# sandialabs/PyNucleus

Measured on AMD Instinct MI355X. Metric: element-pairs/sec assembled (2D P1 fractional s=0.5, dense) + % fp64 roofline, higher is better.
Workload: dtype f64; 1 GPU; 2D unit disc (uniform_disc refined 7x, 98304 cells), P1, 48769 DoFs, fractional s=0.5, horizon=inf, dense getDense incl. zeroExterior; 4831887360 element pairs/step; noRef=7, num_dofs=48769, num_cells=98304, parallelism=block rows of the upper triangle dealt over 1 GPU(s), row-owned one-sided slabs

## Files before the change

include/pnl_hip.h:

```cpp
#ifndef PNL_HIP_H
#define PNL_HIP_H
#include <stdint.h>

#ifdef __cplusplus
extern "C" {
#endif

typedef struct pnl_context pnl_context;

enum pnl_status {
    PNL_OK = 0,
    PNL_ERR_INVALID = -1,
    PNL_ERR_UNSUPPORTED = -2,
    PNL_ERR_HIP = -3,
    PNL_ERR_STATE = -4,
    PNL_ERR_ORDER = -5
};

enum pnl_kernel_type { PNL_FRACTIONAL = 0, PNL_INDICATOR = 1, PNL_PERIDYNAMIC = 2, PNL_GAUSSIAN = 3, PNL_EXPONENTIAL = 4,
                       PNL_GAUSSIAN_BOUNDARY = 5, PNL_EXPONENTIAL_BOUNDARY = 6 };

typedef struct {
    int32_t ktype;
    int32_t interaction;
// ... 48 lines not shown
int pnl_set_classes(pnl_context *ctx, int nclasses, int num_labels, const int32_t *cell_labels_host,
                    const int32_t *facet_labels_host, const int32_t *cls_of_host);
int pnl_set_nonsymmetric(pnl_context *ctx, int on);
int pnl_select_class(pnl_context *ctx, int k);
int pnl_set_kernel(pnl_context *ctx, int which, const pnl_kernel *kernel);
int pnl_set_order_formula(pnl_context *ctx, int which, const pnl_order_formula *formula);
int pnl_upload_distant_rules(pnl_context *ctx, int qmax, const int32_t *off_host, const double *bary_host,
                             const double *w_host, const double *phi_host, const int32_t *foff_host,
                             const double *fbary_host, const double *fw_host);
int pnl_upload_singular_rule(pnl_context *ctx, int which, int panel, int M, int rows, const double *nodes_host,
                             const double *w_host, const double *psi_host, double fac);
int pnl_upload_boundary(pnl_context *ctx, int nb, const int32_t *bcells_host);

int pnl_assemble_pairs_in_horizon(pnl_context *ctx, double *data, double *diag);
int pnl_assemble_pairs_in_horizon_range(pnl_context *ctx, double *data_dev, double *diag_dev, int cell_begin, int cell_end);

#define PNL_FLAG_NO_MIRROR 1
#define PNL_FLAG_SYMMETRIC_FLUSH 2
int pnl_assemble_dense(pnl_context *ctx, double *A_dev, int64_t ldA, int zero_exterior, int cell_begin, int cell_end,
                       int flags);
int pnl_block_row_costs(pnl_context *ctx, double *cost_out, int n);
int pnl_dense_overwrites(pnl_context *ctx, int cell_begin, int cell_end, int flags);
int pnl_tile_cells(pnl_context *ctx);
int pnl_assemble_dense_tiles(pnl_context *ctx, double *A_dev, int64_t ldA, int zero_exterior, int ntiles,
                             const int32_t *tiles_host, int cell_begin, int cell_end, int flags);
int pnl_upload_sparsity(pnl_context *ctx, int nnz, const int32_t *indptr_host, const int32_t *indices_host);
int pnl_upload_sparsity_device(pnl_context *ctx, int nnz, const int32_t *indptr_dev, const int32_t *indices_dev);
int pnl_assemble_pairs_masked(pnl_context *ctx, int np, const int32_t *pairs_host, const uint64_t *masks_host,
                              double *data_dev, double *diag_dev);
int pnl_assemble_boundary_masked(pnl_context *ctx, int ni, const int32_t *cells_host, const int32_t *facets_host,
                                 const uint32_t *masks_host, double fac, double *data_dev, double *diag_dev);
typedef struct {
    int32_t npairs, nnodes, nchunks, chunk_stride, ntiles, num_dslots, nfacets, tile;
    const int32_t *pair_nodes, *node_off, *node_dofs;
    const int32_t *chunk_cells, *chunk_ndof, *chunk_dofs;
    const int16_t *chunk_slot;
    const int32_t *tile_chunkA, *tile_chunkB, *tile_pair, *tile_flags, *tile_dslotA, *tile_dslotB;
    const int32_t *d_cell, *d_pair;
    int32_t n_sing[3];
    int32_t n_btouch;
    const int32_t *sing_items[3];
    const int32_t *pair_foff, *fvid;
    const int32_t *bt_slot, *bt_cell, *bt_facet;
} pnl_cluster_plan;
int pnl_assemble_clusters_tiled(pnl_context *ctx, const pnl_cluster_plan *plan, int cluster_boundary, double *data_dev,
                                double *diag_dev);
// ... 174 lines not shown
```

pynucleus_amd/_lib.py:

```python
import ctypes as C
import os
import numpy as np

_HERE = os.path.dirname(os.path.abspath(__file__))
LIB_PATH = os.environ.get('PNL_LIB', os.path.join(_HERE, 'libpnl_hip.so'))

PNL_OK = 0
PNL_ERR_INVALID = -1
PNL_ERR_UNSUPPORTED = -2
PNL_ERR_HIP = -3
PNL_ERR_STATE = -4
PNL_ERR_ORDER = -5
PNL_INTERIOR = 0
PNL_BOUNDARY = 1
PNL_FLAG_NO_MIRROR = 1
PNL_FLAG_SYMMETRIC_FLUSH = 2
PNL_NUM_COUNTERS = 134

EXPORTS = ['pnl_create', 'pnl_destroy', 'pnl_error_string', 'pnl_version', 'pnl_set_stream', 'pnl_synchronize',
           'pnl_upload_mesh', 'pnl_upload_dofmap', 'pnl_set_kernel', 'pnl_set_order_formula', 'pnl_upload_distant_rules',
           'pnl_upload_singular_rule', 'pnl_upload_boundary', 'pnl_assemble_dense', 'pnl_dense_overwrites', 'pnl_block_row_costs', 'pnl_tile_cells',
           'pnl_assemble_dense_tiles', 'pnl_get_counters', 'pnl_get_phase_ms', 'pnl_get_kernel_ms', 'pnl_tree_build', 'pnl_tree_build_blocks', 'pnl_tree_build_refined', 'pnl_tree_build_horizon', 'pnl_tree_build_device', 'pnl_tree_destroy', 'pnl_tree_sizes', 'pnl_tree_get', 'pnl_tree_node_cells', 'pnl_h2_transfer_matrices', 'pnl_nfplan_build', 'pnl_nfplan_destroy', 'pnl_nfplan_sizes', 'pnl_nfplan_get', 'pnl_horizon_pattern', 'pnl_near_pattern', 'pnl_pattern_set_max_nnz', 'pnl_set_option', 'pnl_set_cell_order', 'pnl_set_interaction_transform', 'pnl_set_order_vertex_values', 'pnl_h2_get', 'pnl_h2_set', 'pnl_pattern_nnz', 'pnl_pattern_get', 'pnl_pattern_destroy', 'pnl_set_row_slab', 'pnl_diag_blocks_size', 'pnl_get_diag_blocks', 'pnl_slab_matvec', 'pnl_slab_diagonal', 'pnl_gemv', 'pnl_cg_jacobi',
           'pnl_inv_diagonal', 'pnl_set_classes', 'pnl_select_class', 'pnl_upload_sparsity', 'pnl_upload_sparsity_device', 'pnl_assemble_pairs_masked', 'pnl_assemble_boundary_masked', 'pnl_assemble_clusters_tiled', 'pnl_h2_setup', 'pnl_h2_matvec', 'pnl_h2_upward', 'pnl_h2_interact', 'pnl_h2_downward', 'pnl_h2_sizes', 'pnl_spmv',
           'pnl_assemble_pairs_in_horizon', 'pnl_assemble_pairs_in_horizon_range', 'pnl_set_nonsymmetric', 'pnl_set_order_function', 'pnl_upload_pointwise_rules', 'pnl_assemble_dense_pointwise',
           'pnl_assemble_pairs_masked_pointwise', 'pnl_assemble_boundary_masked_pointwise',
           'pnl_gemv_axpby', 'pnl_csr_matvec', 'pnl_mg_create', 'pnl_mg_destroy', 'pnl_mg_cycle', 'pnl_mg_solve', 'pnl_mg_cg', 'pnl_theta_step', 'pnl_selftest',
           'pnl_potrf', 'pnl_potrs', 'pnl_getrf', 'pnl_getrs',
           'pnl_csr_cg_jacobi', 'pnl_fe_space_create', 'pnl_fe_space_destroy', 'pnl_assemble_nonlinearity', 'pnl_imex_create',
           'pnl_imex_destroy', 'pnl_imex_sweep']

PNL_FUN_BRUSSELATOR, PNL_FUN_CUBIC = 0, 1
PNL_IMEX_CG_MG, PNL_IMEX_CHOL = 0, 1
PNL_IMEX_MAX_STAGES, PNL_IMEX_MAX_COMP = 4, 2


def source_sha16():
    import glob
    import hashlib
    root = os.path.dirname(_HERE)
    files = sorted(glob.glob(os.path.join(_HERE, 'csrc', '*.h'))+glob.glob(os.path.join(_HERE, 'csrc', '*.hip'))
                   +[os.path.join(root, 'include', 'pnl_hip.h'), os.path.join(_HERE, 'csrc', 'Makefile')])
    h = hashlib.sha256()
    for fn in files:
        with open(fn, 'rb') as f:
# ... 68 lines not shown
    import torch
    L = C.CDLL(LIB_PATH)
    vp, i32, i64, dbl = C.c_void_p, C.c_int, C.c_int64, C.c_double
    L.pnl_create.argtypes = [i32, C.POINTER(vp)]
    L.pnl_destroy.argtypes = [vp]
    L.pnl_destroy.restype = None
    L.pnl_error_string.argtypes = [vp]
    L.pnl_error_string.restype = C.c_char_p
    L.pnl_version.restype = C.c_char_p
    L.pnl_set_stream.argtypes = [vp, vp]
    L.pnl_synchronize.argtypes = [vp]
    L.pnl_upload_mesh.argtypes = [vp, i32, i32, vp, i32, vp, vp, vp, dbl]
    L.pnl_upload_dofmap.argtypes = [vp, i32, i32, i32, i32, vp, vp]
    L.pnl_set_kernel.argtypes = [vp, i32, C.POINTER(pnl_kernel)]
    L.pnl_selftest.argtypes = [i32, i32, i32, i32, vp, i32, vp, vp]
    L.pnl_set_order_formula.argtypes = [vp, i32, C.POINTER(pnl_order_formula)]
    L.pnl_upload_distant_rules.argtypes = [vp, i32, vp, vp, vp, vp, vp, vp, vp]
    L.pnl_upload_singular_rule.argtypes = [vp, i32, i32, i32, i32, vp, vp, vp, dbl]
    L.pnl_upload_boundary.argtypes = [vp, i32, vp]
    L.pnl_assemble_dense.argtypes = [vp, vp, i64, i32, i32, i32, i32]
    L.pnl_dense_overwrites.argtypes = [vp, i32, i32, i32]
    L.pnl_block_row_costs.argtypes = [vp, vp, i32]
    L.pnl_tile_cells.argtypes = [vp]
    L.pnl_assemble_dense_tiles.argtypes = [vp, vp, i64, i32, i32, vp, i32, i32, i32]
    L.pnl_get_counters.argtypes = [vp, vp, i32]
    L.pnl_get_phase_ms.argtypes = [vp, vp, i32]
    L.pnl_get_kernel_ms.argtypes = [vp, vp, i32]
    L.pnl_set_row_slab.argtypes = [vp, i32, vp, i32, vp]
    L.pnl_tree_build.argtypes = [i32, i32, vp, vp, vp, i32, dbl, i32, i32, i32, C.POINTER(vp)]
    L.pnl_tree_build_blocks.argtypes = [i32, i32, vp, vp, vp, i32, dbl, i32, i32, i32, vp, i32, C.POINTER(vp)]
    L.pnl_tree_build_refined.argtypes = [i32, i32, vp, vp, vp, i32, dbl, i32, i32, i32, vp, i32, i32, C.POINTER(vp)]
    L.pnl_tree_build_horizon.argtypes = [i32, i32, vp, vp, vp, i32, dbl, i32, i32, i32, vp, i32, i32, dbl, C.POINTER(vp)]
    L.pnl_tree_build_device.argtypes = [i32, i32, vp, vp, vp, i32, dbl, i32, i32, i32, i32, C.POINTER(vp)]
    L.pnl_tree_destroy.argtypes = [vp]
    L.pnl_tree_destroy.restype = None
    L.pnl_tree_sizes.argtypes = [vp, vp]
    L.pnl_tree_get.argtypes = [vp, vp, vp, vp, vp, vp, vp, vp, vp]
    L.pnl_tree_node_cells.argtypes = [vp, i32, vp, vp, vp]
    L.pnl_h2_transfer_matrices.argtypes = [i32, i32, i32, vp, vp, vp]
    L.pnl_nfplan_build.argtypes = [i32, i32, vp, i32, vp, i32, i32, vp, i32, vp, vp, vp, vp, i32, vp, i32, i32, C.POINTER(vp)]
    L.pnl_nfplan_destroy.argtypes = [vp]
    L.pnl_nfplan_destroy.restype = None
    L.pnl_nfplan_sizes.argtypes = [vp, vp]
    L.pnl_nfplan_get.argtypes = [vp, i32, vp]
    L.pnl_horizon_pattern.argtypes = [i32, i32, vp, i32, vp, i32, i32, vp, dbl, i32, C.POINTER(vp)]
    L.pnl_near_pattern.argtypes = [vp, i32, vp, i32, C.POINTER(vp)]
# ... 242 lines not shown

    def set_stream(self, stream_ptr):
        self.check(self.L.pnl_set_stream(self.h, C.c_void_p(stream_ptr)))

    def synchronize(self):
        self.check(self.L.pnl_synchronize(self.h))

    def assemble_dense(self, A_ptr, ldA, zero_exterior, cell_begin, cell_end, flags=0):
        self.assembly_epoch = getattr(self, 'assembly_epoch', 0)+1
        self.check(self.L.pnl_assemble_dense(self.h, C.c_void_p(A_ptr), int(ldA), int(bool(zero_exterior)), int(cell_begin),
                                             int(cell_end), int(flags)))

    def block_row_costs(self, num_blocks):
        out = np.zeros(int(num_blocks))
        self.check(self.L.pnl_block_row_costs(self.h, out.ctypes.data, int(num_blocks)))
        return out

    def dense_overwrites(self, cell_begin, cell_end, flags=0):
        rc = self.L.pnl_dense_overwrites(self.h, int(cell_begin), int(cell_end), int(flags))
        if rc < 0:
            self.check(rc)
        return rc == 1

    def tile_cells(self):
        rc = self.L.pnl_tile_cells(self.h)
        if rc <= 0:
            self.check(rc)
        return rc

    def assemble_dense_tiles(self, A_ptr, ldA, zero_exterior, tiles, cell_begin, cell_end, flags=0):
        self.assembly_epoch = getattr(self, 'assembly_epoch', 0)+1
        t, pt = _hp(tiles, np.int32)
        self.check(self.L.pnl_assemble_dense_tiles(self.h, C.c_void_p(A_ptr), int(ldA), int(bool(zero_exterior)), t.shape[0], pt,
                                                   int(cell_begin), int(cell_end), int(flags)))

    def upload_sparsity(self, indptr, indices):
        ip, pip = _hp(indptr, np.int32)
        ix, pix = _hp(indices, np.int32)
        self.check(self.L.pnl_upload_sparsity(self.h, ix.shape[0], pip, pix))

    def upload_sparsity_device(self, indptr_t, indices_t):
        self.check(self.L.pnl_upload_sparsity_device(self.h, int(indices_t.numel()), C.c_void_p(indptr_t.data_ptr()),
                                                     C.c_void_p(indices_t.data_ptr()) if indices_t.numel() else None))

    def assemble_pairs_masked(self, pairs, masks, data_ptr, diag_ptr=None):
        p, pp = _hp(pairs, np.int32)
# ... 228 lines not shown
```

pynucleus_amd/csrc/pnl_context.h:

```cpp
#pragma once
#include <hip/hip_runtime.h>
#include <algorithm>
#include <cmath>
#include <cstdarg>
#include <cstdio>
#include <cstring>
#include <string>
#include <vector>
#include "pnl_hip.h"
#include "pnl_device.h"


constexpr int TILE_P1 = 64;
constexpr int TILE_P2 = 32;

struct DevBuf {
    void *p = nullptr;
    size_t bytes = 0;
    ~DevBuf() { release(); }
    void release() { if (p) { (void)hipFree(p); p = nullptr; bytes = 0; } }
};


struct pnl_context {
// ... 24 lines not shown
        int n_spairs[3] = {0, 0, 0}, n_bpairs[2] = {0, 0};
        int n_spairs1[3] = {0, 0, 0};
        ClassData() { std::memset(kern, 0, sizeof(kern)); std::memset(form, 0, sizeof(form)); }
    };
    std::vector<ClassData*> cls;
    int cur = 0;
    ClassData &C() { return *cls[cur]; }
    int nlab = 0;
    bool nonsym = false;
    int orient = 0;
    std::vector<int32_t> cell_labels, facet_labels, cls_of;
    bool have_mesh = false, have_dofs = false, have_rules = false, have_boundary = false;
    bool dirty = true;
    DevProblem P;
    DevBuf b_cellv, b_ccen, b_cvol, b_ch, b_clog, b_cvid, b_cdof, b_cslot, b_blk_ndof, b_blk_dofs, b_perm, b_off, b_bary, b_w, b_phi,
        b_foff, b_fbary, b_fw, b_bvid, b_bv, b_bgeo, b_counters, b_D, b_tiles,
        b_vec[6], b_clabel, b_blabel, b_clsof, b_scal, b_wl, b_wlcount, b_tilectr, b_ttn, b_ttoff, b_tttab, b_ttwphi, b_wlsorted, b_wlaux,
        b_vertices, b_sp_indptr, b_sp_indices, b_mp_pairs, b_mp_masks, b_mp_wl, b_mp_sorted, b_mp_aux, b_bi_cells, b_bi_facets,
        b_bi_masks, b_cp[28], b_cpD, b_wlds, b_wlpair, b_h2[20];
    DevBuf b_kcls, b_fcls, b_uni, b_tilecls, b_ttwphif;
    DevBuf b_scolbase, b_srowoff, b_cpoff, b_cpslot, b_cprow, b_foldtab, b_bkcls, b_bfcls, b_bdefer, b_multitiles, b_slotA, b_candtiles, b_candq;
    int slot_S = 0, n_multitiles = 0;
    long long slot_total = 0;
    DevBuf b_rowmap, b_rowdof, b_colmap, b_coldof;
    DevBuf b_cholinfo;
    DevBuf b_luwork, b_lutmp;
    std::vector<int32_t> slab_rowdofs, slab_coldofs;
    int slab_rows = 0, slab_cols = 0;
    bool slot_full_list = false;
    bool slot_used = false;
    std::vector<DevKernel> kcls_host;
    std::vector<DevKernel> bkcls_host;
    std::vector<DevFormula> bfcls_host;
    std::vector<DevFormula> fcls_host;
    int uni_off[5] = {-1, -1, -1, -1, -1}, uni_np[5] = {0, 0, 0, 0, 0};
    bool uni_struct[5] = {false, false, false, false, false};
    H2Dev h2;
    bool have_h2 = false;
    bool have_tile_order = false;
    struct TileOrderJob *tile_job = nullptr;
    DevBuf b_cellv_t, b_cdof_t, b_cslot_t, b_Dt;
    PwDev pw;
    bool have_pw = false, have_pw_rules[2][3] = {{false, false, false}, {false, false, false}};
    int pw_nkeys[2] = {0, 0};
    std::vector<double> pw_cell_smax, pw_facet_smax;
    std::vector<double> pw_vertex_s;
// ... 205 lines not shown
```

pynucleus_amd/csrc/pnl_device.h:

```cpp
#pragma once
#include <hip/hip_runtime.h>
#include <stdint.h>

#define PNL_NTHREADS 256
#define PNL_MAXQ 120
#define PNL_NCOUNTERS 134
#define PNL_WL_SLOTS 256

struct DevKernel {
    int ktype;
    int fast;
    double exponent, scale, horizon2;
    int interaction, qm;
    double pb[6];
    const double *ptab;
};

struct DevFormula {
    double c0, a, b, e, den0;
    int clip;
    int pad;
};

struct DevProblem {
// ... 30 lines not shown
    const double *sNodes[3], *sW[3], *sPsi[3];
    double sFac;
    int bM[2];
    const double *bNodes[2], *bW[2], *bPhi[2];
    double bFac;
    const int *bvid;
    const double *bv;
    const double *bgeo;
    const int *clabel, *blabel, *cls_of;
    int nlab, cur_class;
    int orient, pad2;
    double idfac;
    unsigned long long *counters;
    const int *rowmap, *colmap;
    int onesided, pad3;
    const double *uni = nullptr;
    int uni_off[5] = {0, 0, 0, 0, 0};
    int mix_struct = 0;
};

__device__ __forceinline__ long long pnl_row(const DevProblem &P, int I) { return P.rowmap ? (long long)P.rowmap[I] : (long long)I; }
__device__ __forceinline__ int pnl_col(const DevProblem &P, int J) { return P.colmap ? P.colmap[J] : J; }

#define PNL_FOLD_TAB 63
struct FoldEntry { long long off; int ar, cy; };

struct H2Dev {
    int dim, m, M, nnodes, nleaves, nfar;
    const double *box;
    const int *parent;
    const int *leaf_node;
    const int *leaf_dof_off, *leaf_dofs;
    const int *leaf_cell_off, *leaf_cells;
    const long long *leaf_val_off;
    const int *far;
    double *V, *K;
    const double *T;
    double *cup, *cdown;
};

__device__ __forceinline__ double cheb_node(double a, double b, int m, int j) {
    return (b-a)*0.5*(cos((2.0*(m-j)-1.0)/(2.0*m)*3.14159265358979323846)+1.0)+a;
}

__device__ __forceinline__ double lagrange1d(double a, double b, int m, int l, double x) {
    const double xl = cheb_node(a, b, m, l);
    double v = 1.;
    for (int k = 0; k < m; k++)
// ... 37 lines not shown
```

pynucleus_amd/csrc/pnl_hip.hip:

```cpp
#include <hip/hip_runtime.h>
#include <algorithm>
#include <cmath>
#include <cstdarg>
#include <cstdio>
#include <cstring>
#include <string>
#include <vector>
#include "pnl_hip.h"
#include "pnl_kernels.h"
#include "pnl_bndtile.h"

#include <thread>
#include "pnl_context.h"
#include "pnl_launch.h"

struct TileOrderJob {
    std::vector<int> cells, lperm;
    int nc = 0, T = 0, nblocks = 0, ncp = 0, dim = 0, dpe = 0;
    std::vector<double> cellv;
    std::vector<int32_t> cdof;
    std::vector<int16_t> cslot;
    std::thread worker;
};

namespace {


// ... 334 lines not shown
        for (int b = 0; b < nblocks; b++) colbase[b+1] = colbase[b]+((blk_ndof[b]+7) & ~7);
        const int S = colbase[nblocks];
        std::vector<long long> rowoff(nblocks, 0);
        long long run = 0;
        for (int a = 0; a < nblocks; a++) { rowoff[a] = run; run += (long long)blk_ndof[a]*(S-colbase[a]); }
        ctx->slot_S = S; ctx->slot_total = run;
        std::vector<int32_t> cpoff(ctx->N+1, 0);
        for (int b = 0; b < nblocks; b++) for (int g : lists[b]) cpoff[g+1]++;
        for (int g = 0; g < ctx->N; g++) cpoff[g+1] += cpoff[g];
        std::vector<int2> cp(cpoff[ctx->N]);
        std::vector<int32_t> fillp(cpoff.begin(), cpoff.end()-1);
        std::vector<long long> cprow(cp.size());
        for (int b = 0; b < nblocks; b++)
            for (size_t r = 0; r < lists[b].size(); r++) {
                const int k = fillp[lists[b][r]]++;
                cp[k] = make_int2(b, colbase[b]+(int)r);
                cprow[k] = rowoff[b]+(long long)r*(S-colbase[b])-colbase[b];
            }
        if ((rc = upload(ctx, ctx->b_cprow, cprow.data(), cprow.size()))) return rc;
        if ((rc = upload(ctx, ctx->b_scolbase, colbase.data(), colbase.size()))) return rc;
        if ((rc = upload(ctx, ctx->b_srowoff, rowoff.data(), rowoff.size()))) return rc;
        if ((rc = upload(ctx, ctx->b_cpoff, cpoff.data(), cpoff.size()))) return rc;
        if ((rc = upload(ctx, ctx->b_cpslot, cp.data(), cp.size()))) return rc;
        const int nranges = (ctx->N+31)/32;
        std::vector<FoldEntry> tab((size_t)nranges*(PNL_FOLD_TAB+1));
        for (int q = 0; q < nranges; q++) {
            FoldEntry *e = &tab[(size_t)q*(PNL_FOLD_TAB+1)];
            const int g0 = cpoff[q*32], g1 = cpoff[std::min(ctx->N, q*32+32)];
            e[0].off = g1-g0; e[0].ar = 0; e[0].cy = 0;
            if (g1-g0 > PNL_FOLD_TAB) continue;
            for (int I = q*32; I < std::min(ctx->N, q*32+32); I++)
                for (int g = cpoff[I]; g < cpoff[I+1]; g++) {
                    FoldEntry &x = e[1+g-g0];
                    x.off = cprow[g]; x.ar = (cp[g].x << 5) | (I-q*32); x.cy = cp[g].y;
                }
        }
        if ((rc = upload(ctx, ctx->b_foldtab, tab.data(), tab.size()))) return rc;
    }
    if ((rc = upload(ctx, ctx->b_perm, ctx->perm_table.data(), ctx->perm_table.size()))) return rc;
    const bool fresh_counters = !ctx->b_counters.p;
    if ((rc = ensure(ctx, ctx->b_counters, sizeof(unsigned long long)*PNL_NCOUNTERS))) return rc;
    if (fresh_counters) HIPCHK(ctx, hipMemset(ctx->b_counters.p, 0, sizeof(unsigned long long)*PNL_NCOUNTERS));
    if ((rc = ensure(ctx, ctx->b_D, sizeof(double)*(size_t)ncp*(dpe*(dpe+1)/2)))) return rc;

    DevProblem &P = ctx->P;
    P.dim = dim; P.dpe = dpe; P.nc = nc; P.ncp = ncp; P.N = ctx->N; P.dpv = ctx->dpv; P.dped = ctx->dped; P.nb = ctx->nb;
    P.H0 = ctx->H0;
    P.cellv = (const double*)ctx->b_cellv.p; P.ccen = (const double*)ctx->b_ccen.p;
    P.cvol = (const double*)ctx->b_cvol.p; P.ch = (const double*)ctx->b_ch.p; P.clog = (const double*)ctx->b_clog.p;
    P.cvid = (const int*)ctx->b_cvid.p; P.cdof = (const int*)ctx->b_cdof.p; P.cslot = (const short*)ctx->b_cslot.p;
    P.blk_ndof = (const int*)ctx->b_blk_ndof.p; P.blk_dofs = (const int*)ctx->b_blk_dofs.p;
    P.blk_stride = nU; P.nblocks = nblocks;
    P.perm_table = (const int*)ctx->b_perm.p;
    P.bvid = (const int*)ctx->b_bvid.p; P.bv = (const double*)ctx->b_bv.p; P.bgeo = (const double*)ctx->b_bgeo.p;
    P.counters = (unsigned long long*)ctx->b_counters.p;
    P.nlab = nlab; P.cur_class = -1; P.orient = 0; P.pad2 = 0; P.idfac = 1.;
    P.clabel = (const int*)ctx->b_clabel.p; P.blabel = (const int*)ctx->b_blabel.p; P.cls_of = (const int*)ctx->b_clsof.p;
    ctx->dirty = false;
    return PNL_OK;
// ... 889 lines not shown
        const double l_self = std::log(dmax/S.hmin), n_other = std::log(dmax/O.hmin);
        const double aL = std::min(F.a*O.Lmin, F.a*O.Lmax);
        const double bL = std::min(F.b*std::max(S.Lmin, O.Lmin), F.b*std::max(S.Lmax, O.Lmax));
        const double num = F.c0+aL+bL-F.e*n_other, den = l_self+F.den0;
        return den > 0. && num >= q*den*(1.+1e-9)+1e-9;
    };
    for (int q = 2; q <= qlimit; q++)
        if (upper(A, B, q) && upper(B, A, q)) {
            if (q == 2) return 2;
            return (lower(A, B, q-1) || lower(B, A, q-1)) ? q : 0;
        }
    return 0;
}

#include <deque>
#include <map>
#include <mutex>
namespace {
std::mutex g_opt_mutex;
std::map<std::string, const std::string*> g_options;
std::deque<std::string> g_option_values;
const char *const k_product_options[] = {"PNL_WL_FRAC", "PNL_FH_NOTILES", "PNL_NO_POWTAB", "PNL_VERBOSE", "PNL_PLAN_TIMING", "PNL_PLAN_THREADS", "PNL_BND_OLD",
                                         "PNL_NO_OVERLAP", "PNL_NO_FORK",
                                         "PNL_TILE_WGS", "PNL_UNI_GENERIC", "PNL_MIXED_GENERIC"};
}

const char *pnl_tune(const char *name) {
    {
        std::lock_guard<std::mutex> lk(g_opt_mutex);
        auto it = g_options.find(name);
        if (it != g_options.end()) return it->second->c_str();
    }
#ifdef PNL_TUNING
    return getenv(name);
#else
    return nullptr;
#endif
}

extern "C" {

const char *pnl_version(void) {
#ifdef PNL_TUNING
    return "pnl_hip 0.1 (gfx950, tuning build)";
#else
    return "pnl_hip 0.1 (gfx950)";
#endif
// ... 364 lines not shown
        if ((rc = upload(ctx, ctx->C().b_sn[slot], nodes, (size_t)2*nV*M))) return rc;
        if ((rc = upload(ctx, ctx->C().b_sw[slot], w, (size_t)M))) return rc;
        if ((rc = upload(ctx, ctx->C().b_sp[slot], psi, (size_t)rows*M))) return rc;
        ctx->C().sM[slot] = M; ctx->C().sRows[slot] = rows; ctx->C().sFac = facv;
    } else {
        if (rows != dpe) return fail(ctx, PNL_ERR_INVALID, "boundary singular rule has %d rows, expected %d", rows, dpe);
        if ((rc = upload(ctx, ctx->C().b_bn[slot], nodes, (size_t)(nV+dim)*M))) return rc;
        if ((rc = upload(ctx, ctx->C().b_bw[slot], w, (size_t)M))) return rc;
        if ((rc = upload(ctx, ctx->C().b_bp[slot], psi, (size_t)rows*M))) return rc;
        ctx->C().bM[slot] = M; ctx->C().bFac = facv;
    }
    ctx->C().have_sing[which][slot] = true;
    return PNL_OK;
}

int pnl_upload_boundary(pnl_context *ctx, int nb, const int32_t *bcells) {
    if (!ctx) return PNL_ERR_INVALID;
    if (!ctx->have_mesh) return fail(ctx, PNL_ERR_STATE, "upload the mesh first");
    if (nb < 0 || (nb > 0 && !bcells)) return fail(ctx, PNL_ERR_INVALID, "bad boundary arguments");
    ctx->nb = nb;
    ctx->bcells.assign(bcells, bcells+(size_t)nb*ctx->dim);
    ctx->have_boundary = true;
    ctx->dirty = true;
    return PNL_OK;
}

int pnl_tile_cells(pnl_context *ctx) {
    if (!ctx) return PNL_ERR_INVALID;
    int rc = finalize(ctx);
    return rc ? rc : ctx->tile;
}

static int upload_tiles(pnl_context *ctx, std::vector<int2> &tiles, int cell_begin, int cell_end) {
    const int ncls = (int)ctx->cls.size();
    std::vector<pnl_order_formula> forms(ncls);
    for (int k = 0; k < ncls; k++) forms[k] = ctx->cls[k]->form[0];
    if (tiles.size() == ctx->tiles_cached.size() && ctx->b_tiles.p && ctx->tiles_cb == cell_begin && ctx->tiles_ce == cell_end &&
        forms.size() == ctx->tiles_forms.size() && std::memcmp(forms.data(), ctx->tiles_forms.data(), sizeof(pnl_order_formula)*ncls) == 0 &&
        ctx->tiles_filter == ctx->tile_cell_filter &&
        (tiles.empty() || std::memcmp(tiles.data(), ctx->tiles_cached.data(), tiles.size()*sizeof(int2)) == 0))
        return PNL_OK;
    const int T = ctx->tile;
    const bool filter = ctx->tile_cell_filter;
    const bool p1 = T == 64 && (ctx->dpe == 3 || ctx->dpe == 2), p2 = ctx->dim == 2 && ctx->dpe == 6;
    const bool allow = ctx->use_pure && (p1 || p2) && ctx->qmax >= 2 && !ctx->nonsym;
    int qlimit = 2;
// ... 554 lines not shown
```

pynucleus_amd/csrc/pnl_tile2.h:

```cpp
#pragma once
#include "pnl_common.h"

__host__ __device__ constexpr int uni_rule_size(int dpe, int np) { return 3*np+np+np*dpe+(dpe*(dpe+1)/2)*np; }


#ifndef PNL_FOLD_FLAT
#define PNL_FOLD_FLAT 1
#endif
template <bool NT>
__global__ void __launch_bounds__(256)
k_fold_mirror(const double *__restrict__ A2, const FoldEntry *__restrict__ tab, const int *__restrict__ cpoff, const int2 *__restrict__ cp,
              const long long *__restrict__ cprow, double *__restrict__ A, long long ldA, int N) {
    __shared__ double t1[32][33], t2[32][33];
    __shared__ FoldEntry s_tab[2][PNL_FOLD_TAB+1];
    const unsigned nb = (unsigned)(N+31)/32;
    const unsigned nbs = (nb+7)/8;
    const unsigned sbid = blockIdx.x >> 6, inner = blockIdx.x & 63;
    unsigned I;
    {
        const float t = 2.f*(float)nbs+1.f;
        const float fb = (t-sqrtf(fmaxf(t*t-8.f*(float)sbid, 0.f)))*0.5f;
        I = (unsigned)fmaxf(fb, 0.f);
        if (I >= nbs) I = nbs-1;
        while (I > 0 && I*nbs-I*(I-1)/2 > sbid) I--;
        while (I+1 < nbs && (I+1)*nbs-(I+1)*I/2 <= sbid) I++;
    }
    const unsigned J = I+(sbid-(I*nbs-I*(I-1)/2));
    const unsigned bi = 8*I+(inner >> 3), bj = 8*J+(inner & 7);
    if (bi > bj || bj >= nb) return;
    const int tid = threadIdx.x, tx = tid & 31, ty = tid >> 5;
    if (tid < 2*(PNL_FOLD_TAB+1)) {
        const int side = tid >= PNL_FOLD_TAB+1, k = tid-side*(PNL_FOLD_TAB+1);
        s_tab[side][k] = tab[(size_t)(side ? bj : bi)*(PNL_FOLD_TAB+1)+k];
    }
    for (int k = tid; k < 32*33; k += 256) { (&t1[0][0])[k] = 0.; (&t2[0][0])[k] = 0.; }
    __syncthreads();
    const int n0 = (int)s_tab[0][0].off, n1 = (int)s_tab[1][0].off;
    if (n0 <= PNL_FOLD_TAB && n1 <= PNL_FOLD_TAB) {
#if PNL_FOLD_FLAT
#pragma unroll
        for (int g = 0; g < 2; g++) {
            if (g && bi == bj) break;
            const int nr = g ? n1 : n0, nc = g ? n0 : n1;
            double *__restrict__ tf = g ? &t2[0][0] : &t1[0][0];
            const unsigned total = (unsigned)(nr*nc), inv = ((1u << 20)+(unsigned)nc-1u)/(unsigned)nc;
            for (unsigned base = 0; base < total; base += 8*256) {
                double v[8];
                int dst[8];
#pragma unroll
                for (int u = 0; u < 8; u++) {
                    const unsigned idx = base+256u*u+(unsigned)tid;
                    dst[u] = -1;
                    v[u] = 0.;
                    if (idx < total) {
                        const unsigned ci = (idx*inv) >> 20, cj = idx-ci*(unsigned)nc;
                        const FoldEntry rw = s_tab[g][1+ci], col = s_tab[1-g][1+cj];
                        if ((col.ar >> 5) >= (rw.ar >> 5)) { v[u] = A2[rw.off+col.cy]; dst[u] = (rw.ar & 31)*33+(col.ar & 31); }
                    }
                }
#pragma unroll
                for (int u = 0; u < 8; u++) if (dst[u] >= 0) lds_add_f64(tf+dst[u], v[u]);
            }
        }
#else
#pragma unroll
        for (int g = 0; g < 2; g++) {
            if (g && bi == bj) break;
            const int nr = g ? n1 : n0, nc = g ? n0 : n1;
            double *__restrict__ tf = g ? &t2[0][0] : &t1[0][0];
            for (int cj = tx; cj < nc; cj += 32) {
                const FoldEntry col = s_tab[1-g][1+cj];
                const int cb = col.ar >> 5, c = col.ar & 31;
                for (int ci0 = ty; ci0 < nr; ci0 += 48) {
                    double v[6];
                    int dst[6];
#pragma unroll
                    for (int u = 0; u < 6; u++) {
                        const int ci = ci0+8*u;
                        dst[u] = -1;
                        v[u] = 0.;
                        if (ci < nr) {
                            const FoldEntry rw = s_tab[g][1+ci];
                            if (cb >= (rw.ar >> 5)) { v[u] = A2[rw.off+col.cy]; dst[u] = (rw.ar & 31)*33+c; }
                        }
                    }
#pragma unroll
                    for (int u = 0; u < 6; u++) if (dst[u] >= 0) lds_add_f64(tf+dst[u], v[u]);
                }
            }
        }
#endif
    } else {
        auto gather = [&](int br, int bc, double (*t)[33]) {
            const int J = min(bc*32+tx, N), j0 = cpoff[J], j1 = cpoff[min(J+1, N)];
#pragma unroll 1
            for (int rr = 0; rr < 4; rr++) {
                const int r = ty+8*rr, I = min(br*32+r, N);
                double s = 0.;
                for (int ci = cpoff[I]; ci < cpoff[min(I+1, N)]; ci++) {
                    const int a = cp[ci].x;
                    const double *__restrict__ rowp = A2+cprow[ci];
                    for (int cj = j0; cj < j1; cj++) {
                        const int2 c2 = cp[cj];
                        if (c2.x >= a) s += rowp[c2.y];
                    }
                }
                t[r][tx] = s;
            }
        };
        gather((int)bi, (int)bj, t1);
        if (bi != bj) gather((int)bj, (int)bi, t2);
    }
    __syncthreads();
    for (int r = ty; r < 32; r += 8) {
        const int I = bi*32+r, J = bj*32+tx;
        if (I < N && J < N) {
            const double v = (bi != bj) ? t1[r][tx]+t2[tx][r] : ((r != tx) ? t1[r][tx]+t1[tx][r] : t1[r][tx]);
            if (NT) __builtin_nontemporal_store(v, A+(long long)I*ldA+J); else A[(long long)I*ldA+J] = v;
        }
        const int I2 = bj*32+r, J2 = bi*32+tx;
        if (bi != bj && I2 < N && J2 < N) {
            const double v = t2[r][tx]+t1[tx][r];
            if (NT) __builtin_nontemporal_store(v, A+(long long)I2*ldA+J2); else A[(long long)I2*ldA+J2] = v;
        }
    }
}

__global__ void __launch_bounds__(256)
k_zero_slot_tiles(const SlotOut SO, const int2 *__restrict__ tiles, const int *__restrict__ blk_ndof) {
    const int a = tiles[blockIdx.x].x, b = tiles[blockIdx.x].y;
    const int nA = blk_ndof[a], nBp = SO.colbase[b+1]-SO.colbase[b], W = SO.S-SO.colbase[a];
    double *__restrict__ base = SO.A2+SO.rowoff[a]+(SO.colbase[b]-SO.colbase[a]);
    for (int t = threadIdx.x; t < nA*nBp; t += 256) {
        const int r = t/nBp, c = t-r*nBp;
        base[(long long)r*W+c] = 0.;
    }
}

__host__ __device__ constexpr size_t uniform_fixed_lds(int dpe, int np, int tile, int nUe, bool dof_lists = true) {
    return dpe == 3 ? sizeof(double)*(size_t)(2*tile*(np*2+1)+2*tile+2*tile*(np|1)+(dpe*(dpe+1)/2)*np)
                      +sizeof(int)*(size_t)(2*tile*(dpe|1)+2*tile+(dof_lists ? 4*nUe : 0))
                    : sizeof(double)*(size_t)(tile*np*2+tile*6+2*tile+2*tile*np+(dpe*(dpe+1)/2)*np)
                      +sizeof(int)*(size_t)(2*tile*dpe+2*tile+(dof_lists ? 4*nUe : 0));
}

// ... 976 lines not shown
```

pynucleus_amd/csrc/pnl_tile2.hip:

```cpp
#include "pnl_context.h"
#include "pnl_tile2.h"

namespace {

template <int DPE, int NP, int KT, bool STRUCT = false>
int launch_uniform_t(pnl_context *ctx, const DevProblem &Pt, const int2 *tiles, const int *tile_cls, int ntiles, int q, double *A,
                     int64_t ldA, double *Dglob, const SlotOut &SO) {
    constexpr int TILE = DPE == 6 ? 32 : 64;
    const int nUe = (ctx->nU+1) & ~1;
    const size_t fixed = uniform_fixed_lds(DPE, NP, TILE, nUe, SO.A2 == nullptr);
    int acc_stride = nUe+1;
    while (acc_stride % 32 != 1) acc_stride++;
    if (fixed+sizeof(double)*(size_t)(nUe+1)*acc_stride > 80*1024) acc_stride = (nUe+1) | 1;
    size_t lds = fixed+sizeof(double)*(size_t)(nUe+1)*acc_stride;
    if (lds > 160*1024)
        return fail(ctx, PNL_ERR_UNSUPPORTED, "a block of %d cells touches %d DoFs: LDS sub-block of %zu bytes exceeds 160 KiB", TILE, ctx->nU, lds);
    const size_t cap_cu = (size_t)std::max(1, pnl_tune("PNL_UNI_PER_CU") ? atoi(pnl_tune("PNL_UNI_PER_CU")) : 4);
    auto kfun = k_tile_uniform<DPE, NP, KT, STRUCT>;
    HIPCHK(ctx, hipFuncSetAttribute((const void*)kfun, hipFuncAttributeMaxDynamicSharedMemorySize, (int)std::min<size_t>(160*1024, lds+sizeof(double)*PNL_POW_TAB_DOUBLES)));
    auto resident = [&](size_t bytes) -> int {
        int occ = 0;
        if (hipOccupancyMaxActiveBlocksPerMultiprocessor(&occ, (const void*)kfun, 256, bytes) != hipSuccess || occ < 1) {
            (void)hipGetLastError();
            occ = (int)std::min<size_t>(2, (160*1024)/bytes);
// ... 82 lines not shown
    if (ctx->dpe == 6 && np == 6) return launch_uniform_kt<6, 6>(ctx, kt, Pt, tiles, tile_cls, ntiles, q, A, ldA, Dglob, SO);
    if (ctx->dpe == 3 && np == 6) return launch_uniform_kt<3, 6>(ctx, kt, Pt, tiles, tile_cls, ntiles, q, A, ldA, Dglob, SO);
    if (ctx->dpe == 3 && np == 3) return launch_uniform_kt<3, 3>(ctx, kt, Pt, tiles, tile_cls, ntiles, q, A, ldA, Dglob, SO);
    return fail(ctx, PNL_ERR_UNSUPPORTED, "uniform tiles: dpe=%d with %d points", ctx->dpe, np);
}

int pnl2_launch_p2(pnl_context *ctx, int kt, const int2 *tiles, const int *tile_cls, int ntiles, double *A, int64_t ldA,
                   int cell_begin, int cell_end, unsigned wl_cap_each, const SlotOut &SO) {
    if (ntiles <= 0) return PNL_OK;
    if (kt == 2) return launch_p2_t<2>(ctx, tiles, tile_cls, ntiles, A, ldA, cell_begin, cell_end, wl_cap_each, SO);
    if (kt == 1) return launch_p2_t<1>(ctx, tiles, tile_cls, ntiles, A, ldA, cell_begin, cell_end, wl_cap_each, SO);
    return launch_p2_t<0>(ctx, tiles, tile_cls, ntiles, A, ldA, cell_begin, cell_end, wl_cap_each, SO);
}

int pnl2_zero_slot_tiles(pnl_context *ctx, const SlotOut &SO) {
    if (ctx->n_multitiles <= 0) return PNL_OK;
    hipLaunchKernelGGL(k_zero_slot_tiles, dim3(ctx->n_multitiles), dim3(256), 0, ctx->stream, SO, (const int2*)ctx->b_multitiles.p,
                       (const int*)ctx->b_blk_ndof.p);
    HIPCHK(ctx, hipGetLastError());
    return PNL_OK;
}

int pnl2_fold_mirror(pnl_context *ctx, const SlotOut &SO, double *A, int64_t ldA) {
    const long long nb = (ctx->N+31)/32, nbs = (nb+7)/8;
    if (nbs*(nbs+1)/2*64 >= (1ll << 31)) return fail(ctx, PNL_ERR_UNSUPPORTED, "fold pass: %d DoFs exceed the grid size", ctx->N);
    kt_begin(ctx, PNL_K_FOLD_MIRROR);
    hipLaunchKernelGGL(k_fold_mirror<true>, dim3((unsigned)(nbs*(nbs+1)/2*64)), dim3(256), 0, ctx->stream, (const double*)SO.A2, (const FoldEntry*)ctx->b_foldtab.p, (const int*)ctx->b_cpoff.p,
                       (const int2*)ctx->b_cpslot.p, (const long long*)ctx->b_cprow.p, A, (long long)ldA, ctx->N);
    kt_end(ctx, PNL_K_FOLD_MIRROR);
    HIPCHK(ctx, hipGetLastError());
    return PNL_OK;
}
```

Before: 57.50 billion element-pairs/s.

## Rework fold-mirror kernel with 64-wide tiles, paired column loads and single LDS tile

```diff
diff --git a/include/pnl_hip.h b/include/pnl_hip.h
--- a/include/pnl_hip.h
+++ b/include/pnl_hip.h
@@ -94,6 +94,7 @@
 int pnl_block_row_costs(pnl_context *ctx, double *cost_out, int n);
 int pnl_dense_overwrites(pnl_context *ctx, int cell_begin, int cell_end, int flags);
 int pnl_tile_cells(pnl_context *ctx);
+int pnl_fold_ranges(pnl_context *ctx, int32_t *packed, int32_t *total);
 int pnl_assemble_dense_tiles(pnl_context *ctx, double *A_dev, int64_t ldA, int zero_exterior, int ntiles,
                              const int32_t *tiles_host, int cell_begin, int cell_end, int flags);
 int pnl_upload_sparsity(pnl_context *ctx, int nnz, const int32_t *indptr_host, const int32_t *indices_host);
diff --git a/pynucleus_amd/_lib.py b/pynucleus_amd/_lib.py
--- a/pynucleus_amd/_lib.py
+++ b/pynucleus_amd/_lib.py
@@ -19,7 +19,7 @@
 
 EXPORTS = ['pnl_create', 'pnl_destroy', 'pnl_error_string', 'pnl_version', 'pnl_set_stream', 'pnl_synchronize',
            'pnl_upload_mesh', 'pnl_upload_dofmap', 'pnl_set_kernel', 'pnl_set_order_formula', 'pnl_upload_distant_rules',
-           'pnl_upload_singular_rule', 'pnl_upload_boundary', 'pnl_assemble_dense', 'pnl_dense_overwrites', 'pnl_block_row_costs', 'pnl_tile_cells',
+           'pnl_upload_singular_rule', 'pnl_upload_boundary', 'pnl_assemble_dense', 'pnl_dense_overwrites', 'pnl_block_row_costs', 'pnl_tile_cells', 'pnl_fold_ranges',
            'pnl_assemble_dense_tiles', 'pnl_get_counters', 'pnl_get_phase_ms', 'pnl_get_kernel_ms', 'pnl_tree_build', 'pnl_tree_build_blocks', 'pnl_tree_build_refined', 'pnl_tree_build_horizon', 'pnl_tree_build_device', 'pnl_tree_destroy', 'pnl_tree_sizes', 'pnl_tree_get', 'pnl_tree_node_cells', 'pnl_h2_transfer_matrices', 'pnl_nfplan_build', 'pnl_nfplan_destroy', 'pnl_nfplan_sizes', 'pnl_nfplan_get', 'pnl_horizon_pattern', 'pnl_near_pattern', 'pnl_pattern_set_max_nnz', 'pnl_set_option', 'pnl_set_cell_order', 'pnl_set_interaction_transform', 'pnl_set_order_vertex_values', 'pnl_h2_get', 'pnl_h2_set', 'pnl_pattern_nnz', 'pnl_pattern_get', 'pnl_pattern_destroy', 'pnl_set_row_slab', 'pnl_diag_blocks_size', 'pnl_get_diag_blocks', 'pnl_slab_matvec', 'pnl_slab_diagonal', 'pnl_gemv', 'pnl_cg_jacobi',
            'pnl_inv_diagonal', 'pnl_set_classes', 'pnl_select_class', 'pnl_upload_sparsity', 'pnl_upload_sparsity_device', 'pnl_assemble_pairs_masked', 'pnl_assemble_boundary_masked', 'pnl_assemble_clusters_tiled', 'pnl_h2_setup', 'pnl_h2_matvec', 'pnl_h2_upward', 'pnl_h2_interact', 'pnl_h2_downward', 'pnl_h2_sizes', 'pnl_spmv',
            'pnl_assemble_pairs_in_horizon', 'pnl_assemble_pairs_in_horizon_range', 'pnl_set_nonsymmetric', 'pnl_set_order_function', 'pnl_upload_pointwise_rules', 'pnl_assemble_dense_pointwise',
@@ -134,6 +134,7 @@
     L.pnl_dense_overwrites.argtypes = [vp, i32, i32, i32]
     L.pnl_block_row_costs.argtypes = [vp, vp, i32]
     L.pnl_tile_cells.argtypes = [vp]
+    L.pnl_fold_ranges.argtypes = [vp, vp, vp]
     L.pnl_assemble_dense_tiles.argtypes = [vp, vp, i64, i32, i32, vp, i32, i32, i32]
     L.pnl_get_counters.argtypes = [vp, vp, i32]
     L.pnl_get_phase_ms.argtypes = [vp, vp, i32]
@@ -422,6 +423,11 @@
             self.check(rc)
         return rc == 1
 
+    def fold_ranges(self):
+        packed, total = C.c_int32(0), C.c_int32(0)
+        self.check(self.L.pnl_fold_ranges(self.h, C.byref(packed), C.byref(total)))
+        return packed.value, total.value
+
     def tile_cells(self):
         rc = self.L.pnl_tile_cells(self.h)
         if rc <= 0:
diff --git a/pynucleus_amd/csrc/pnl_context.h b/pynucleus_amd/csrc/pnl_context.h
--- a/pynucleus_amd/csrc/pnl_context.h
+++ b/pynucleus_amd/csrc/pnl_context.h
@@ -70,6 +70,7 @@
     DevBuf b_scolbase, b_srowoff, b_cpoff, b_cpslot, b_cprow, b_foldtab, b_bkcls, b_bfcls, b_bdefer, b_multitiles, b_slotA, b_candtiles, b_candq;
     int slot_S = 0, n_multitiles = 0;
     long long slot_total = 0;
+    int fold_ranges = 0, fold_packed = 0;
     DevBuf b_rowmap, b_rowdof, b_colmap, b_coldof;
     DevBuf b_cholinfo;
     DevBuf b_luwork, b_lutmp;
diff --git a/pynucleus_amd/csrc/pnl_device.h b/pynucleus_amd/csrc/pnl_device.h
--- a/pynucleus_amd/csrc/pnl_device.h
+++ b/pynucleus_amd/csrc/pnl_device.h
@@ -76,8 +76,16 @@
 __device__ __forceinline__ long long pnl_row(const DevProblem &P, int I) { return P.rowmap ? (long long)P.rowmap[I] : (long long)I; }
 __device__ __forceinline__ int pnl_col(const DevProblem &P, int J) { return P.colmap ? P.colmap[J] : J; }
 
-#define PNL_FOLD_TAB 63
-struct FoldEntry { long long off; int ar, cy; };
+#define PNL_FOLD_B 64
+#define PNL_FOLD_ROWS 128
+#define PNL_FOLD_PAIRS 96
+struct alignas(16) FoldRange {
+    int nrows, npairs, pad0, pad1;
+    long long off[PNL_FOLD_ROWS];
+    int ar[PNL_FOLD_ROWS];
+    int2 pr[PNL_FOLD_PAIRS];
+};
+static_assert(sizeof(FoldRange) % 16 == 0, "k_fold_mirror copies a FoldRange in 16-byte pieces");
 
 struct H2Dev {
     int dim, m, M, nnodes, nleaves, nfar;
diff --git a/pynucleus_amd/csrc/pnl_hip.hip b/pynucleus_amd/csrc/pnl_hip.hip
--- a/pynucleus_amd/csrc/pnl_hip.hip
+++ b/pynucleus_amd/csrc/pnl_hip.hip
@@ -3,6 +3,7 @@
 #include <cmath>
 #include <cstdarg>
 #include <cstdio>
+#include <cstdlib>
 #include <cstring>
 #include <string>
 #include <vector>
@@ -383,19 +384,43 @@
         if ((rc = upload(ctx, ctx->b_srowoff, rowoff.data(), rowoff.size()))) return rc;
         if ((rc = upload(ctx, ctx->b_cpoff, cpoff.data(), cpoff.size()))) return rc;
         if ((rc = upload(ctx, ctx->b_cpslot, cp.data(), cp.size()))) return rc;
-        const int nranges = (ctx->N+31)/32;
-        std::vector<FoldEntry> tab((size_t)nranges*(PNL_FOLD_TAB+1));
+        int cap_rows = PNL_FOLD_ROWS, cap_pairs = PNL_FOLD_PAIRS;
+        if (const char *e = pnl_tune("PNL_FOLD_CAP")) {
+            const int v = std::atoi(e);
+            cap_rows = std::max(0, std::min(cap_rows, v)); cap_pairs = std::max(0, std::min(cap_pairs, v));
+        }
+        if (nblocks >= (1 << 17)) cap_rows = -1;
+        const int nranges = (ctx->N+PNL_FOLD_B-1)/PNL_FOLD_B;
+        std::vector<FoldRange> tab((size_t)nranges);
+        int npacked = 0;
+        std::vector<std::pair<int, int>> cols;
         for (int q = 0; q < nranges; q++) {
-            FoldEntry *e = &tab[(size_t)q*(PNL_FOLD_TAB+1)];
-            const int g0 = cpoff[q*32], g1 = cpoff[std::min(ctx->N, q*32+32)];
-            e[0].off = g1-g0; e[0].ar = 0; e[0].cy = 0;
-            if (g1-g0 > PNL_FOLD_TAB) continue;
-            for (int I = q*32; I < std::min(ctx->N, q*32+32); I++)
+            FoldRange &e = tab[q];
+            std::memset(&e, 0, sizeof(e));
+            const int I0 = q*PNL_FOLD_B, I1 = std::min(ctx->N, I0+PNL_FOLD_B), g0 = cpoff[I0], g1 = cpoff[I1];
+            e.nrows = -1;
+            if (g1-g0 > cap_rows) continue;
+            cols.clear();
+            for (int I = I0; I < I1; I++)
                 for (int g = cpoff[I]; g < cpoff[I+1]; g++) {
-                    FoldEntry &x = e[1+g-g0];
-                    x.off = cprow[g]; x.ar = (cp[g].x << 5) | (I-q*32); x.cy = cp[g].y;
+                    e.off[g-g0] = cprow[g]; e.ar[g-g0] = (cp[g].x << 6) | (I-I0);
+                    cols.emplace_back(cp[g].y, (cp[g].x << 6) | (I-I0));
                 }
-        }
+            std::sort(cols.begin(), cols.end());
+            int np = 0;
+            bool fits = true;
+            for (size_t k = 0; k < cols.size();) {
+                const int cy = cols[k].first & ~1, blk = cols[k].second >> 6;
+                int l0 = PNL_FOLD_B, l1 = PNL_FOLD_B;
+                for (; k < cols.size() && (cols[k].first & ~1) == cy; k++) ((cols[k].first & 1) ? l1 : l0) = cols[k].second & (PNL_FOLD_B-1);
+                if (np == cap_pairs) { fits = false; break; }
+                e.pr[np++] = make_int2(cy, (blk << 14) | (l1 << 7) | l0);
+            }
+            if (!fits) continue;
+            e.nrows = g1-g0; e.npairs = np;
+            npacked++;
+        }
+        ctx->fold_ranges = nranges; ctx->fold_packed = npacked;
         if ((rc = upload(ctx, ctx->b_foldtab, tab.data(), tab.size()))) return rc;
     }
     if ((rc = upload(ctx, ctx->b_perm, ctx->perm_table.data(), ctx->perm_table.size()))) return rc;
@@ -1331,7 +1356,8 @@
 std::deque<std::string> g_option_values;
 const char *const k_product_options[] = {"PNL_WL_FRAC", "PNL_FH_NOTILES", "PNL_NO_POWTAB", "PNL_VERBOSE", "PNL_PLAN_TIMING", "PNL_PLAN_THREADS", "PNL_BND_OLD",
                                          "PNL_NO_OVERLAP", "PNL_NO_FORK",
-                                         "PNL_TILE_WGS", "PNL_UNI_GENERIC", "PNL_MIXED_GENERIC"};
+                                         "PNL_TILE_WGS", "PNL_UNI_GENERIC", "PNL_MIXED_GENERIC",
+                                         "PNL_FOLD_CAP"};
 }
 
 const char *pnl_tune(const char *name) {
@@ -1742,6 +1768,14 @@
     ctx->bcells.assign(bcells, bcells+(size_t)nb*ctx->dim);
     ctx->have_boundary = true;
     ctx->dirty = true;
+    return PNL_OK;
+}
+
+int pnl_fold_ranges(pnl_context *ctx, int32_t *packed, int32_t *total) {
+    if (!ctx || !packed || !total) return PNL_ERR_INVALID;
+    int rc = finalize(ctx);
+    if (rc) return rc;
+    *packed = ctx->fold_packed; *total = ctx->fold_ranges;
     return PNL_OK;
 }
 
diff --git a/pynucleus_amd/csrc/pnl_tile2.h b/pynucleus_amd/csrc/pnl_tile2.h
--- a/pynucleus_amd/csrc/pnl_tile2.h
+++ b/pynucleus_amd/csrc/pnl_tile2.h
@@ -4,22 +4,25 @@
 __host__ __device__ constexpr int uni_rule_size(int dpe, int np) { return 3*np+np+np*dpe+(dpe*(dpe+1)/2)*np; }
 
 
-#ifndef PNL_FOLD_FLAT
-#define PNL_FOLD_FLAT 1
+#ifndef PNL_FOLD_U
+#define PNL_FOLD_U 6
 #endif
 template <bool NT>
-__global__ void __launch_bounds__(256)
-k_fold_mirror(const double *__restrict__ A2, const FoldEntry *__restrict__ tab, const int *__restrict__ cpoff, const int2 *__restrict__ cp,
+__global__ void __launch_bounds__(512)
+k_fold_mirror(const double *__restrict__ A2, const FoldRange *__restrict__ tab, const int *__restrict__ cpoff, const int2 *__restrict__ cp,
               const long long *__restrict__ cprow, double *__restrict__ A, long long ldA, int N) {
-    __shared__ double t1[32][33], t2[32][33];
-    __shared__ FoldEntry s_tab[2][PNL_FOLD_TAB+1];
-    const unsigned nb = (unsigned)(N+31)/32;
+    constexpr int B = PNL_FOLD_B, LD = B+1;
+    static_assert(B == 64, "local DoFs are packed in 6 (rows) and 7 (column pairs) bits, the store loop takes 64 columns per wave");
+    __shared__ double t[B*LD];
+    __shared__ FoldRange s_tab[2];
+    const unsigned nb = (unsigned)(N+B-1)/B;
     const unsigned nbs = (nb+7)/8;
-    const unsigned sbid = blockIdx.x >> 6, inner = blockIdx.x & 63;
+    const unsigned wg = (blockIdx.x & 7u)*(gridDim.x >> 3)+(blockIdx.x >> 3);
+    const unsigned sbid = wg >> 6, inner = wg & 63;
     unsigned I;
     {
-        const float t = 2.f*(float)nbs+1.f;
-        const float fb = (t-sqrtf(fmaxf(t*t-8.f*(float)sbid, 0.f)))*0.5f;
+        const float tt = 2.f*(float)nbs+1.f;
+        const float fb = (tt-sqrtf(fmaxf(tt*tt-8.f*(float)sbid, 0.f)))*0.5f;
         I = (unsigned)fmaxf(fb, 0.f);
         if (I >= nbs) I = nbs-1;
         while (I > 0 && I*nbs-I*(I-1)/2 > sbid) I--;
@@ -28,99 +31,97 @@
     const unsigned J = I+(sbid-(I*nbs-I*(I-1)/2));
     const unsigned bi = 8*I+(inner >> 3), bj = 8*J+(inner & 7);
     if (bi > bj || bj >= nb) return;
-    const int tid = threadIdx.x, tx = tid & 31, ty = tid >> 5;
-    if (tid < 2*(PNL_FOLD_TAB+1)) {
-        const int side = tid >= PNL_FOLD_TAB+1, k = tid-side*(PNL_FOLD_TAB+1);
-        s_tab[side][k] = tab[(size_t)(side ? bj : bi)*(PNL_FOLD_TAB+1)+k];
-    }
-    for (int k = tid; k < 32*33; k += 256) { (&t1[0][0])[k] = 0.; (&t2[0][0])[k] = 0.; }
+    const bool diag = bi == bj;
+    const int tid = threadIdx.x, tx = tid & 63, ty = tid >> 6;
+    {
+        constexpr int Q = (int)(sizeof(FoldRange)/16);
+        for (int k = tid; k < 2*Q; k += 512) {
+            const int side = k >= Q;
+            ((int4*)s_tab)[k] = ((const int4*)(tab+(side ? bj : bi)))[k-side*Q];
+        }
+    }
+    for (int k = tid; k < B*LD; k += 512) t[k] = 0.;
     __syncthreads();
-    const int n0 = (int)s_tab[0][0].off, n1 = (int)s_tab[1][0].off;
-    if (n0 <= PNL_FOLD_TAB && n1 <= PNL_FOLD_TAB) {
-#if PNL_FOLD_FLAT
+    if (s_tab[0].nrows >= 0 && s_tab[1].nrows >= 0) {
 #pragma unroll
         for (int g = 0; g < 2; g++) {
-            if (g && bi == bj) break;
-            const int nr = g ? n1 : n0, nc = g ? n0 : n1;
-            double *__restrict__ tf = g ? &t2[0][0] : &t1[0][0];
-            const unsigned total = (unsigned)(nr*nc), inv = ((1u << 20)+(unsigned)nc-1u)/(unsigned)nc;
-            for (unsigned base = 0; base < total; base += 8*256) {
-                double v[8];
-                int dst[8];
-#pragma unroll
-                for (int u = 0; u < 8; u++) {
-                    const unsigned idx = base+256u*u+(unsigned)tid;
+            if (g && diag) break;
+            const FoldRange &R = s_tab[g], &C = s_tab[1-g];
+            const unsigned nr = (unsigned)R.nrows, np = (unsigned)C.npairs, total = nr*np;
+            const unsigned inv = (unsigned)((0x100000000ull+np-1u)/(np > 1u ? np : 2u));
+            for (unsigned base = 0; base < total; base += PNL_FOLD_U*512) {
+                double2 v[PNL_FOLD_U];
+                int dst[PNL_FOLD_U];
+#pragma unroll
+                for (int u = 0; u < PNL_FOLD_U; u++) {
+                    const unsigned idx = base+512u*u+(unsigned)tid;
                     dst[u] = -1;
-                    v[u] = 0.;
+                    v[u] = make_double2(0., 0.);
                     if (idx < total) {
-                        const unsigned ci = (idx*inv) >> 20, cj = idx-ci*(unsigned)nc;
-                        const FoldEntry rw = s_tab[g][1+ci], col = s_tab[1-g][1+cj];
-                        if ((col.ar >> 5) >= (rw.ar >> 5)) { v[u] = A2[rw.off+col.cy]; dst[u] = (rw.ar & 31)*33+(col.ar & 31); }
-                    }
-                }
-#pragma unroll
-                for (int u = 0; u < 8; u++) if (dst[u] >= 0) lds_add_f64(tf+dst[u], v[u]);
-            }
-        }
-#else
-#pragma unroll
-        for (int g = 0; g < 2; g++) {
-            if (g && bi == bj) break;
-            const int nr = g ? n1 : n0, nc = g ? n0 : n1;
-            double *__restrict__ tf = g ? &t2[0][0] : &t1[0][0];
-            for (int cj = tx; cj < nc; cj += 32) {
-                const FoldEntry col = s_tab[1-g][1+cj];
-                const int cb = col.ar >> 5, c = col.ar & 31;
-                for (int ci0 = ty; ci0 < nr; ci0 += 48) {
-                    double v[6];
-                    int dst[6];
-#pragma unroll
-                    for (int u = 0; u < 6; u++) {
-                        const int ci = ci0+8*u;
-                        dst[u] = -1;
-                        v[u] = 0.;
-                        if (ci < nr) {
-                            const FoldEntry rw = s_tab[g][1+ci];
-                            if (cb >= (rw.ar >> 5)) { v[u] = A2[rw.off+col.cy]; dst[u] = (rw.ar & 31)*33+c; }
+                        const unsigned ci = np > 1u ? __umulhi(idx, inv) : idx, pj = idx-ci*np;
+                        const int ar = R.ar[ci];
+                        const int2 pr = C.pr[pj];
+                        if ((pr.y >> 14) >= (ar >> 6)) {
+                            v[u] = *(const double2*)(A2+R.off[ci]+pr.x);
+                            dst[u] = ((ar & 63) << 16) | ((pr.y & 0x3fff) << 1 & 0xff00) | (pr.y & 127);
                         }
                     }
-#pragma unroll
-                    for (int u = 0; u < 6; u++) if (dst[u] >= 0) lds_add_f64(tf+dst[u], v[u]);
-                }
-            }
-        }
-#endif
+                }
+#pragma unroll
+                for (int u = 0; u < PNL_FOLD_U; u++)
+                    if (dst[u] >= 0) {
+                        const int r = dst[u] >> 16, c0 = dst[u] & 255, c1 = (dst[u] >> 8) & 255;
+                        if (c0 < B) {
+                            lds_add_f64(t+(g ? c0*LD+r : r*LD+c0), v[u].x);
+                            if (diag && c0 != r) lds_add_f64(t+c0*LD+r, v[u].x);
+                        }
+                        if (c1 < B) {
+                            lds_add_f64(t+(g ? c1*LD+r : r*LD+c1), v[u].y);
+                            if (diag && c1 != r) lds_add_f64(t+c1*LD+r, v[u].y);
+                        }
+                    }
+            }
+        }
     } else {
-        auto gather = [&](int br, int bc, double (*t)[33]) {
-            const int J = min(bc*32+tx, N), j0 = cpoff[J], j1 = cpoff[min(J+1, N)];
-#pragma unroll 1
-            for (int rr = 0; rr < 4; rr++) {
-                const int r = ty+8*rr, I = min(br*32+r, N);
-                double s = 0.;
-                for (int ci = cpoff[I]; ci < cpoff[min(I+1, N)]; ci++) {
+        auto gather = [&](int br, int bc, double *s) {
+            const int Jc = min(bc*B+tx, N), j0 = cpoff[Jc], j1 = cpoff[min(Jc+1, N)];
+#pragma unroll 1
+            for (int rr = 0; rr < B/8; rr++) {
+                const int Ir = min(br*B+ty+8*rr, N);
+                double acc = 0.;
+                for (int ci = cpoff[Ir]; ci < cpoff[min(Ir+1, N)]; ci++) {
                     const int a = cp[ci].x;
                     const double *__restrict__ rowp = A2+cprow[ci];
                     for (int cj = j0; cj < j1; cj++) {
                         const int2 c2 = cp[cj];
-                        if (c2.x >= a) s += rowp[c2.y];
+                        if (c2.x >= a) acc += rowp[c2.y];
                     }
                 }
-                t[r][tx] = s;
+                s[rr] = acc;
             }
         };
-        gather((int)bi, (int)bj, t1);
-        if (bi != bj) gather((int)bj, (int)bi, t2);
+        double s[B/8];
+        gather((int)bi, (int)bj, s);
+        for (int rr = 0; rr < B/8; rr++) t[(ty+8*rr)*LD+tx] = s[rr];
+        if (!diag) gather((int)bj, (int)bi, s);
+        __syncthreads();
+        if (diag) for (int rr = 0; rr < B/8; rr++) s[rr] = (ty+8*rr != tx) ? t[tx*LD+ty+8*rr] : 0.;
+        __syncthreads();
+        for (int rr = 0; rr < B/8; rr++) {
+            if (diag) t[(ty+8*rr)*LD+tx] += s[rr];
+            else t[tx*LD+ty+8*rr] += s[rr];
+        }
     }
     __syncthreads();
-    for (int r = ty; r < 32; r += 8) {
-        const int I = bi*32+r, J = bj*32+tx;
-        if (I < N && J < N) {
-            const double v = (bi != bj) ? t1[r][tx]+t2[tx][r] : ((r != tx) ? t1[r][tx]+t1[tx][r] : t1[r][tx]);
-            if (NT) __builtin_nontemporal_store(v, A+(long long)I*ldA+J); else A[(long long)I*ldA+J] = v;
-        }
-        const int I2 = bj*32+r, J2 = bi*32+tx;
-        if (bi != bj && I2 < N && J2 < N) {
-            const double v = t2[r][tx]+t1[tx][r];
+    for (int r = ty; r < B; r += 8) {
+        const int Ig = bi*B+r, Jg = bj*B+tx;
+        if (Ig < N && Jg < N) {
+            const double v = t[r*LD+tx];
+            if (NT) __builtin_nontemporal_store(v, A+(long long)Ig*ldA+Jg); else A[(long long)Ig*ldA+Jg] = v;
+        }
+        const int I2 = bj*B+r, J2 = bi*B+tx;
+        if (!diag && I2 < N && J2 < N) {
+            const double v = t[tx*LD+r];
             if (NT) __builtin_nontemporal_store(v, A+(long long)I2*ldA+J2); else A[(long long)I2*ldA+J2] = v;
         }
     }
diff --git a/pynucleus_amd/csrc/pnl_tile2.hip b/pynucleus_amd/csrc/pnl_tile2.hip
--- a/pynucleus_amd/csrc/pnl_tile2.hip
+++ b/pynucleus_amd/csrc/pnl_tile2.hip
@@ -128,10 +128,10 @@
 }
 
 int pnl2_fold_mirror(pnl_context *ctx, const SlotOut &SO, double *A, int64_t ldA) {
-    const long long nb = (ctx->N+31)/32, nbs = (nb+7)/8;
+    const long long nb = (ctx->N+PNL_FOLD_B-1)/PNL_FOLD_B, nbs = (nb+7)/8;
     if (nbs*(nbs+1)/2*64 >= (1ll << 31)) return fail(ctx, PNL_ERR_UNSUPPORTED, "fold pass: %d DoFs exceed the grid size", ctx->N);
     kt_begin(ctx, PNL_K_FOLD_MIRROR);
-    hipLaunchKernelGGL(k_fold_mirror<true>, dim3((unsigned)(nbs*(nbs+1)/2*64)), dim3(256), 0, ctx->stream, (const double*)SO.A2, (const FoldEntry*)ctx->b_foldtab.p, (const int*)ctx->b_cpoff.p,
+    hipLaunchKernelGGL(k_fold_mirror<true>, dim3((unsigned)(nbs*(nbs+1)/2*64)), dim3(512), 0, ctx->stream, (const double*)SO.A2, (const FoldRange*)ctx->b_foldtab.p, (const int*)ctx->b_cpoff.p,
                        (const int2*)ctx->b_cpslot.p, (const long long*)ctx->b_cprow.p, A, (long long)ldA, ctx->N);
     kt_end(ctx, PNL_K_FOLD_MIRROR);
     HIPCHK(ctx, hipGetLastError());
```

Result: faster. 58.54 billion element-pairs/s (median of 6 runs) (+1.8%).
